# mokemokechicken/reversi-alpha-zero

Measured on NVIDIA H100. Metric: self_play_games_per_sec, higher is better.
Workload: dtype f16

## Files before the change

### reversi-alpha-zero_b200/csrc/rz_net_tc.cu

```cuda
#include <stdlib.h>
#include <type_traits>
#include "rz_bitboard.cuh"
#include "rz_net.cuh"
#include "rz_tc_common.cuh"

namespace rz {
namespace tc {

constexpr uint32_t kProducerRegs = 40, kMathRegs = 232;
constexpr int kMathThreads = 256;
constexpr uint32_t kActCg = 2896, kActSlot = 144;
constexpr uint32_t kActBytes = 32 * kActCg;
constexpr uint32_t kStageBytes = 32768, kStages = 3;
constexpr int kResAhead = 4;
constexpr uint32_t kA0Bytes = 8192, kW0Bytes = 16384;
constexpr uint32_t kOffAct = 0;
constexpr uint32_t kOffW = kOffAct + kActBytes;
constexpr uint32_t kOffA0 = kOffW + kStages * kStageBytes;
constexpr uint32_t kOffW0 = kOffA0 + kA0Bytes;
constexpr uint32_t kOffSS = kOffW0 + kW0Bytes;
constexpr uint32_t kOffHw = kOffSS + 2 * 2048;
constexpr uint32_t kOffBar = kOffHw + 768 * 4;
constexpr uint32_t kNumBars = 2 * kStages + 1;
constexpr uint32_t kSmemBytes = kOffBar + kNumBars * 8;
constexpr uint32_t kSmemAlloc = kSmemBytes + 128;
static_assert(kSmemAlloc <= 232448, "shared memory budget exceeded");
static_assert(kTowerResFloatsPerCta == (size_t)kMathThreads * 128, "residual scratch per CTA");

#ifdef RZ_TOWER_STAMPS
enum : int {
    kStTiles,
    kStTile,
    kStKLoop,
    kStFull,
    kStMma,
    kStEpiBar,
    kStEpi0,
    kStEpi1,
    kStEpi2,
    kStEpiLast,
    kStFeat,
    kStEmpty,
    kStCount
};
constexpr int kStMaxCtas = 1024;
__device__ unsigned long long g_tower_stamps[kStMaxCtas][kStCount];
__device__ __forceinline__ void stamp_add(int phase, uint32_t cycles) { atomicAdd(&g_tower_stamps[blockIdx.x][phase], (unsigned long long)cycles); }
#define RZ_STAMP(...) __VA_ARGS__
#else
#define RZ_STAMP(...)
#endif

template <int CL>
__global__ void __launch_bounds__(kThreads, 1) net_tower_kernel(const Params pp) {
    Params p = pp;
    if (p.n_dev) p.n = *p.n_dev;
    extern __shared__ uint8_t smem_raw[];
    const uint32_t base = (smem_u32(smem_raw) + 127u) & ~127u;
    uint8_t* sm = smem_raw + (base - smem_u32(smem_raw));
    const int warp = threadIdx.x >> 5, lane = threadIdx.x & 31;
    const uint32_t bar0 = base + kOffBar;
    auto bar_full = [&](uint32_t s) { return bar0 + s * 8; };
    auto bar_empty = [&](uint32_t s) { return bar0 + (kStages + s) * 8; };
    const uint32_t bar_w0 = bar0 + 2 * kStages * 8;
    const uint32_t ntiles = (p.n + 1) >> 1;
    const int L = p.n_layers;
    const uint32_t crank = CL > 1 ? cluster_ctarank() : 0u;
    const uint32_t cbase = blockIdx.x - crank;
    const uint32_t iters = cbase < ntiles ? (ntiles - cbase + gridDim.x - 1) / gridDim.x : 0u;

    for (uint32_t i = threadIdx.x * 16; i < kActBytes; i += kThreads * 16) *reinterpret_cast<uint4*>(sm + kOffAct + i) = make_uint4(0, 0, 0, 0);
    fence_proxy_async();
    for (uint32_t i = threadIdx.x; i < 768; i += kThreads)
        reinterpret_cast<float*>(sm + kOffHw)[i] = __ldg(i < 512 ? p.blob + p.off_policy_conv + i : p.blob + p.off_value_conv + (i - 512));
    if (threadIdx.x == 0) {
        for (uint32_t s = 0; s < kStages; ++s) { mbar_init(bar_full(s), 1); mbar_init(bar_empty(s), 8 * CL); }
        mbar_init(bar_w0, 1);
        asm volatile("fence.mbarrier_init.release.cluster;" ::: "memory");
    }
    __syncthreads();
    if (CL > 1) cluster_sync_all();

    if (warp >= 8) {
        asm volatile("setmaxnreg.dec.sync.aligned.u32 %0;" ::"n"(kProducerRegs));
        if (warp == 8 && lane == 0) {
            if (iters > 0) {
                mbar_expect_tx(bar_w0, kW0Bytes);
                bulk_g2s(base + kOffW0, p.w0, kW0Bytes, bar_w0);
            }
            uint32_t stage = 0, phase = 0;
            for (uint32_t it = 0; it < iters; ++it) {
                for (int l = 1; l < L; ++l) {
                    const uint8_t* src = reinterpret_cast<const uint8_t*>(p.w) + (size_t)(l - 1) * 36 * kStageBytes;
                    RZ_STAMP(uint32_t st_empty = 0;)
                    for (int s = 0; s < 36; ++s) {
                        RZ_STAMP(const uint32_t c0 = (uint32_t)clock();)
                        mbar_wait(bar_empty(stage), phase ^ 1);
                        RZ_STAMP(st_empty += (uint32_t)clock() - c0;)
                        mbar_expect_tx(bar_full(stage), kStageBytes);
                        if (CL == 1) {
                            bulk_g2s(base + kOffW + stage * kStageBytes, src + (size_t)s * kStageBytes, kStageBytes, bar_full(stage));
                        } else {
                            constexpr uint32_t kSlice = kStageBytes / CL;
                            bulk_g2s_mc(base + kOffW + stage * kStageBytes + crank * kSlice, src + (size_t)s * kStageBytes + crank * kSlice,
                                        kSlice, bar_full(stage), (uint16_t)((1u << CL) - 1u));
                        }
                        if (++stage == kStages) { stage = 0; phase ^= 1; }
                    }
                    RZ_STAMP(stamp_add(kStEmpty, st_empty);)
                }
            }
        }
    } else {
        asm volatile("setmaxnreg.inc.sync.aligned.u32 %0;" ::"n"(kMathRegs));
        const int et = threadIdx.x;
        const int wg = warp >> 2;
        const int r0 = wg * 64 + (warp & 3) * 16 + (lane >> 2);
        const int g0 = r0 >> 3, x = r0 & 7, y = g0 >> 1;
        const int cq = 2 * (lane & 3);
        const uint32_t act_row0 = base + kOffAct + (g0 + 2) * kActSlot + (x + 1) * 16 + cq * 2;
        const uint32_t act_row1 = act_row0 + kActSlot;
        const uint32_t a_wg = base + kOffAct + wg * 8 * kActSlot;
        float* ss_s = reinterpret_cast<float*>(sm + kOffSS);
        float4* res = reinterpret_cast<float4*>(p.res + (size_t)blockIdx.x * kTowerResFloatsPerCta) + et;
        const float* hw = reinterpret_cast<const float*>(sm + kOffHw);
        uint32_t stage = 0, phase = 0, ss_buf = 0;
        float d[128];
        ss_s[et] = __ldg(p.ss + et);
        ss_s[256 + et] = __ldg(p.ss + 256 + et);

        for (uint32_t it = 0; it < iters; ++it) {
            const uint32_t tile = blockIdx.x + it * gridDim.x;
            const uint32_t pos0 = tile * 2;
            RZ_STAMP(const uint32_t st_tile0 = (uint32_t)clock();)
            {
                const int m = et & 127, g = m >> 3, brd = g & 1;
                const bool valid = pos0 + brd < p.n;
                build_layer0_operand(sm + kOffA0, valid ? p.own[pos0 + brd] : 0, valid ? p.enemy[pos0 + brd] : 0, 2 * (et >> 7), g, m & 7,
                                     g >> 1);
                fence_proxy_async();
            }
            float hs[6];
            for (int l = 0; l < L; ++l) {
                const float* sc = ss_s + ss_buf * 512;
                const bool is_conv2 = l > 0 && (l & 1) == 0;
                float4 rb[kResAhead];
                RZ_STAMP(uint32_t st_c = (uint32_t)clock(), st_bar = 0, st_full = 0, st_mma = 0;)
                epi_bar();
                RZ_STAMP(st_bar += (uint32_t)clock() - st_c;)
                {
                    const size_t nl = l + 1 < L ? (size_t)l + 1 : 0;
                    const uint32_t dst = smem_u32(ss_s + (ss_buf ^ 1) * 512 + et);
                    cp_async_4(dst, p.ss + nl * 512 + et);
                    cp_async_4(dst + 1024, p.ss + nl * 512 + 256 + et);
                }
                RZ_STAMP(const uint32_t st_k0 = (uint32_t)clock();)
                acc_fence(d);
                if (l == 0) {
                    RZ_STAMP(st_c = (uint32_t)clock();)
                    mbar_wait(bar_w0, 0);
                    RZ_STAMP(st_full += (uint32_t)clock() - st_c;)
                    wgmma_fence();
#pragma unroll
                    for (uint32_t j = 0; j < 2; ++j)
                        wgmma_m64n256k16(d, smem_desc(base + kOffA0 + j * 2 * 2048 + wg * 1024, 2048, 128),
                                         smem_desc(base + kOffW0 + j * 2 * 4096, 4096, 128), j);
                    wgmma_commit();
                    RZ_STAMP(st_c = (uint32_t)clock();)
                    wgmma_wait<0>();
                    RZ_STAMP(st_mma += (uint32_t)clock() - st_c;)
                } else {
                    int prev = -1;
                    for (uint32_t tap = 0; tap < 9; ++tap) {
                        const uint32_t a_tap = a_wg + (2 * (tap / 3)) * kActSlot + (tap % 3) * 16;
                        for (uint32_t kb = 0; kb < 4; ++kb) {
                            RZ_STAMP(st_c = (uint32_t)clock();)
                            mbar_wait(bar_full(stage), phase);
                            RZ_STAMP(st_full += (uint32_t)clock() - st_c;)
                            const uint32_t b_st = base + kOffW + stage * kStageBytes;
                            wgmma_fence();
#pragma unroll
                            for (uint32_t j = 0; j < 4; ++j)
                                wgmma_m64n256k16(d, smem_desc(a_tap + (kb * 8 + 2 * j) * kActCg, kActCg, kActSlot),
                                                 smem_desc(b_st + 2 * j * 4096, 4096, 128), (tap | kb | j) != 0);
                            wgmma_commit();
                            RZ_STAMP(st_c = (uint32_t)clock();)
                            wgmma_wait<1>();
                            RZ_STAMP(st_mma += (uint32_t)clock() - st_c;)
                            if (prev >= 0 && lane == 0) {
                                mbar_arrive(bar_empty(prev));
                                if (CL > 1) mbar_arrive_cta(bar_empty(prev), crank ^ 1u);
                            }
                            prev = (int)stage;
                            if (++stage == kStages) { stage = 0; phase ^= 1; }
                        }
                    }
                    if (is_conv2) {
#pragma unroll
                        for (int i = 0; i < kResAhead; ++i) rb[i] = res[i * 256];
                    }
                    RZ_STAMP(st_c = (uint32_t)clock();)
                    wgmma_wait<0>();
                    RZ_STAMP(st_mma += (uint32_t)clock() - st_c;)
                    if (lane == 0) {
                        mbar_arrive(bar_empty(prev));
                        if (CL > 1) mbar_arrive_cta(bar_empty(prev), crank ^ 1u);
                    }
                }
                RZ_STAMP(const uint32_t st_k1 = (uint32_t)clock();)
                acc_fence(d);
                cp_async_wait_all();
                ss_buf ^= 1;
                const bool keep_res = l == 0 || is_conv2;
                const bool last = l == L - 1;
                RZ_STAMP(st_c = (uint32_t)clock();)
                if (!last) epi_bar();
                RZ_STAMP(const uint32_t st_e0 = (uint32_t)clock(); st_bar += st_e0 - st_c;)
                float* dbg0 = nullptr;
                float* dbg1 = nullptr;
                if (last && p.dbg_tower) {
                    if (pos0 < p.n) dbg0 = p.dbg_tower + ((size_t)pos0 * 64 + y * 8 + x) * 256;
                    if (pos0 + 1 < p.n) dbg1 = p.dbg_tower + ((size_t)(pos0 + 1) * 64 + y * 8 + x) * 256;
                }
                constexpr int kEpiRelu = 0, kEpiKeep = 1, kEpiLast = 2;
                auto epilogue = [&](auto conv2, auto kind) {
                    constexpr bool kConv2 = decltype(conv2)::value;
                    constexpr bool kKeep = decltype(kind)::value == kEpiKeep, kLast = decltype(kind)::value == kEpiLast;
                    if (kLast) {
#pragma unroll
                        for (int k = 0; k < 6; ++k) hs[k] = 0.f;
                    }
#pragma unroll
                for (int i = 0; i < 32; ++i) {
                    const int c = 8 * i + cq;
                    const float2 s = *reinterpret_cast<const float2*>(sc + c);
                    const float2 b = *reinterpret_cast<const float2*>(sc + 256 + c);
                    float v0 = fmaf(d[4 * i + 0], s.x, b.x), v1 = fmaf(d[4 * i + 1], s.y, b.y);
                    float v2 = fmaf(d[4 * i + 2], s.x, b.x), v3 = fmaf(d[4 * i + 3], s.y, b.y);
                    if (kConv2) {
                        const float4 r = rb[i % kResAhead];
                        if (i + kResAhead < 32) rb[i % kResAhead] = res[(i + kResAhead) * 256];
                        v0 += r.x; v1 += r.y; v2 += r.z; v3 += r.w;
                    }
                    if (kKeep || kLast) {
                        v0 = fmaxf(v0, 0.f); v1 = fmaxf(v1, 0.f); v2 = fmaxf(v2, 0.f); v3 = fmaxf(v3, 0.f);
                    }
                    if (!kLast) {
                        if (kKeep) res[i * 256] = make_float4(v0, v1, v2, v3);
                        const uint32_t h0 = pack_h2<!kKeep>(v0, v1);
                        const uint32_t h1 = pack_h2<!kKeep>(v2, v3);
                        const uint32_t off = (c >> 3) * kActCg;
                        asm volatile("st.shared.b32 [%0], %1;" ::"r"(act_row0 + off), "r"(h0) : "memory");
                        asm volatile("st.shared.b32 [%0], %1;" ::"r"(act_row1 + off), "r"(h1) : "memory");
                    } else {
                        const float4 w = *reinterpret_cast<const float4*>(hw + 2 * c);
                        const float2 wv = *reinterpret_cast<const float2*>(hw + 512 + c);
                        hs[0] = fmaf(v1, w.z, fmaf(v0, w.x, hs[0]));
                        hs[1] = fmaf(v1, w.w, fmaf(v0, w.y, hs[1]));
                        hs[2] = fmaf(v1, wv.y, fmaf(v0, wv.x, hs[2]));
                        hs[3] = fmaf(v3, w.z, fmaf(v2, w.x, hs[3]));
                        hs[4] = fmaf(v3, w.w, fmaf(v2, w.y, hs[4]));
                        hs[5] = fmaf(v3, wv.y, fmaf(v2, wv.x, hs[5]));
                        if (dbg0) *reinterpret_cast<float2*>(dbg0 + c) = make_float2(v0, v1);
                        if (dbg1) *reinterpret_cast<float2*>(dbg1 + c) = make_float2(v2, v3);
                    }
                }
                };
                using Conv2 = std::true_type;
                using NoConv2 = std::false_type;
                if (last) {
                    if (is_conv2) epilogue(Conv2(), std::integral_constant<int, kEpiLast>());
                    else epilogue(NoConv2(), std::integral_constant<int, kEpiLast>());
                } else if (is_conv2) {
                    epilogue(Conv2(), std::integral_constant<int, kEpiKeep>());
                } else if (keep_res) {
                    epilogue(NoConv2(), std::integral_constant<int, kEpiKeep>());
                } else {
                    epilogue(NoConv2(), std::integral_constant<int, kEpiRelu>());
                }
                if (!last) fence_proxy_async();
                RZ_STAMP(if (et == 0) {
                    stamp_add(kStKLoop, st_k1 - st_k0); stamp_add(kStFull, st_full); stamp_add(kStMma, st_mma); stamp_add(kStEpiBar, st_bar);
                    stamp_add(l == 0 ? kStEpi0 : last ? kStEpiLast : is_conv2 ? kStEpi2 : kStEpi1, (uint32_t)clock() - st_e0);
                })
            }
            RZ_STAMP(const uint32_t st_h0 = (uint32_t)clock();)
#pragma unroll
            for (int k = 0; k < 6; ++k) {
                hs[k] += __shfl_xor_sync(0xffffffffu, hs[k], 1);
                hs[k] += __shfl_xor_sync(0xffffffffu, hs[k], 2);
            }
            {
                const int q = lane & 3;
                if (q < 2 && pos0 + q < p.n) {
                    const float h0 = q ? hs[3] : hs[0], h1 = q ? hs[4] : hs[1], h2 = q ? hs[5] : hs[2];
                    store_head_features(p.feat + (size_t)(pos0 + q) * kHeadFeatures, p.ss + (size_t)L * 512, y * 8 + x, h0 + 0.f,
                                        h1 + 0.f, h2 + 0.f);
                }
            }
            RZ_STAMP(if (et == 0) {
                const uint32_t st_h1 = (uint32_t)clock();
                stamp_add(kStFeat, st_h1 - st_h0); stamp_add(kStTile, st_h1 - st_tile0); stamp_add(kStTiles, 1);
            })
        }
    }

    __syncthreads();
    if (CL > 1) cluster_sync_all();
}

int launch_tower(const Params& p, cudaStream_t stream) {
    return launch_tower_pairs<net_tower_kernel<1>, net_tower_kernel<2>, kSmemAlloc, 2>(p, stream);
}

}

static int g_cluster = 0;

int set_tower_cluster(int cluster) {
    RZ_REQUIRE(cluster == 1 || cluster == 2, "rz_net_set_tower_cluster: cluster must be 1 or 2");
    g_cluster = cluster;
    return RZ_OK;
}

int tower_cluster() {
    if (g_cluster == 0) {
        const char* cs = getenv("RZ_TOWER_CLUSTER");
        g_cluster = (cs && atoi(cs) == 1) ? 1 : 2;
    }
    return g_cluster;
}

}

#ifdef RZ_TOWER_STAMPS
extern "C" int rz_tower_stamps(unsigned long long* out, int n_ctas, int reset) {
    using namespace rz::tc;
    if (n_ctas < 0 || n_ctas > kStMaxCtas) return (int)cudaErrorInvalidValue;
    const size_t bytes = (size_t)n_ctas * kStCount * sizeof(unsigned long long);
    cudaError_t e = cudaDeviceSynchronize();
    if (e == cudaSuccess && out) e = cudaMemcpyFromSymbol(out, g_tower_stamps, bytes);
    if (e == cudaSuccess && reset) {
        void* dev = nullptr;
        e = cudaGetSymbolAddress(&dev, g_tower_stamps);
        if (e == cudaSuccess) e = cudaMemset(dev, 0, sizeof(g_tower_stamps));
        if (e == cudaSuccess) e = cudaDeviceSynchronize();
    }
    return (int)e;
}
extern "C" int rz_tower_stamp_count() { return rz::tc::kStCount; }
#endif
```

### reversi-alpha-zero_b200/csrc/rz_tc_common.cuh

```cuda
#pragma once
#include <cuda_fp16.h>
#include "rz_bitboard.cuh"
#include "rz_net.cuh"

namespace rz {
namespace tc {

__device__ __forceinline__ uint32_t smem_u32(const void* p) { return (uint32_t)__cvta_generic_to_shared(p); }

__device__ __forceinline__ void mbar_init(uint32_t bar, uint32_t count) {
    asm volatile("mbarrier.init.shared::cta.b64 [%0], %1;" ::"r"(bar), "r"(count) : "memory");
}
__device__ __forceinline__ void mbar_expect_tx(uint32_t bar, uint32_t bytes) {
    asm volatile("mbarrier.arrive.expect_tx.shared::cta.b64 _, [%0], %1;" ::"r"(bar), "r"(bytes) : "memory");
}
__device__ __forceinline__ void mbar_arrive(uint32_t bar) {
    asm volatile("mbarrier.arrive.shared::cta.b64 _, [%0];" ::"r"(bar) : "memory");
}
__device__ __forceinline__ void mbar_arrive_cta(uint32_t bar, uint32_t rank) {
    uint32_t remote;
    asm volatile("mapa.shared::cluster.u32 %0, %1, %2;" : "=r"(remote) : "r"(bar), "r"(rank));
    asm volatile("mbarrier.arrive.shared::cluster.b64 _, [%0];" ::"r"(remote) : "memory");
}
__device__ __forceinline__ void mbar_wait(uint32_t bar, uint32_t parity) {
    uint32_t ok = 0;
    long long t0 = 0;
    for (uint32_t spin = 0; !ok; ++spin) {
        asm volatile(
            "{\n\t.reg .pred p;\n\t"
            "mbarrier.try_wait.parity.shared::cta.b64 p, [%1], %2;\n\t"
            "selp.u32 %0, 1, 0, p;\n\t}"
            : "=r"(ok)
            : "r"(bar), "r"(parity)
            : "memory");
        if (!ok && (spin & 1023) == 1023) {
            const long long now = clock64();
            if (t0 == 0) t0 = now;
            else if (now - t0 > 8000000000LL) __trap();
        }
    }
}
__device__ __forceinline__ void bulk_g2s(uint32_t dst, const void* src, uint32_t bytes, uint32_t bar) {
    asm volatile("cp.async.bulk.shared::cluster.global.mbarrier::complete_tx::bytes [%0], [%1], %2, [%3];" ::"r"(dst), "l"(src),
                 "r"(bytes), "r"(bar)
                 : "memory");
}
__device__ __forceinline__ void bulk_g2s_mc(uint32_t dst, const void* src, uint32_t bytes, uint32_t bar, uint16_t mask) {
    asm volatile(
        "cp.async.bulk.shared::cluster.global.mbarrier::complete_tx::bytes.multicast::cluster [%0], [%1], %2, [%3], %4;" ::"r"(dst),
        "l"(src), "r"(bytes), "r"(bar), "h"(mask)
        : "memory");
}
__device__ __forceinline__ void cluster_sync_all() {
    asm volatile("barrier.cluster.arrive.release.aligned;\n\tbarrier.cluster.wait.acquire.aligned;" ::: "memory");
}
__device__ __forceinline__ uint32_t cluster_ctarank() {
    uint32_t r;
    asm volatile("mov.u32 %0, %%cluster_ctarank;" : "=r"(r));
    return r;
}
__device__ __forceinline__ void cp_async_4(uint32_t dst, const void* src) {
    asm volatile("cp.async.ca.shared.global [%0], [%1], 4;" ::"r"(dst), "l"(src) : "memory");
}
__device__ __forceinline__ void cp_async_wait_all() { asm volatile("cp.async.wait_all;" ::: "memory"); }
__device__ __forceinline__ void fence_proxy_async() { asm volatile("fence.proxy.async.shared::cta;" ::: "memory"); }
__device__ __forceinline__ void epi_bar() { asm volatile("bar.sync 1, 256;" ::: "memory"); }

__device__ __forceinline__ uint64_t smem_desc(uint32_t addr, uint32_t lbo, uint32_t sbo) {
    return (uint64_t)((addr >> 4) & 0x3FFF) | ((uint64_t)((lbo >> 4) & 0x3FFF) << 16) | ((uint64_t)((sbo >> 4) & 0x3FFF) << 32);
}
__device__ __forceinline__ void wgmma_fence() { asm volatile("wgmma.fence.sync.aligned;" ::: "memory"); }
__device__ __forceinline__ void wgmma_commit() { asm volatile("wgmma.commit_group.sync.aligned;" ::: "memory"); }
template <int N>
__device__ __forceinline__ void wgmma_wait() { asm volatile("wgmma.wait_group.sync.aligned %0;" ::"n"(N) : "memory"); }
__device__ __forceinline__ void acc_fence(float (&d)[128]) {
#pragma unroll
    for (int i = 0; i < 128; ++i) asm volatile("" : "+f"(d[i])::"memory");
}

#define RZ_D4(i) "+f"(d[i]), "+f"(d[i + 1]), "+f"(d[i + 2]), "+f"(d[i + 3])
#define RZ_D16(i) RZ_D4(i), RZ_D4(i + 4), RZ_D4(i + 8), RZ_D4(i + 12)
__device__ __forceinline__ void wgmma_m64n256k16(float (&d)[128], uint64_t adesc, uint64_t bdesc, uint32_t accumulate) {
    asm volatile(
        "{\n\t.reg .pred p;\n\t"
        "setp.ne.b32 p, %130, 0;\n\t"
        "wgmma.mma_async.sync.aligned.m64n256k16.f32.f16.f16 {"
        "%0, %1, %2, %3, %4, %5, %6, %7, %8, %9, %10, %11, %12, %13, %14, %15, "
        "%16, %17, %18, %19, %20, %21, %22, %23, %24, %25, %26, %27, %28, %29, %30, %31, "
        "%32, %33, %34, %35, %36, %37, %38, %39, %40, %41, %42, %43, %44, %45, %46, %47, "
        "%48, %49, %50, %51, %52, %53, %54, %55, %56, %57, %58, %59, %60, %61, %62, %63, "
        "%64, %65, %66, %67, %68, %69, %70, %71, %72, %73, %74, %75, %76, %77, %78, %79, "
        "%80, %81, %82, %83, %84, %85, %86, %87, %88, %89, %90, %91, %92, %93, %94, %95, "
        "%96, %97, %98, %99, %100, %101, %102, %103, %104, %105, %106, %107, %108, %109, %110, %111, "
        "%112, %113, %114, %115, %116, %117, %118, %119, %120, %121, %122, %123, %124, %125, %126, %127"
        "}, %128, %129, p, 1, 1, 0, 0;\n\t}"
        : RZ_D16(0), RZ_D16(16), RZ_D16(32), RZ_D16(48), RZ_D16(64), RZ_D16(80), RZ_D16(96), RZ_D16(112)
        : "l"(adesc), "l"(bdesc), "r"(accumulate)
        : "memory");
}
template <int O>
__device__ __forceinline__ void wgmma_m64n128k16(float (&d)[128], uint64_t adesc, uint64_t bdesc, uint32_t accumulate) {
    asm volatile(
        "{\n\t.reg .pred p;\n\t"
        "setp.ne.b32 p, %66, 0;\n\t"
        "wgmma.mma_async.sync.aligned.m64n128k16.f32.f16.f16 {"
        "%0, %1, %2, %3, %4, %5, %6, %7, %8, %9, %10, %11, %12, %13, %14, %15, "
        "%16, %17, %18, %19, %20, %21, %22, %23, %24, %25, %26, %27, %28, %29, %30, %31, "
        "%32, %33, %34, %35, %36, %37, %38, %39, %40, %41, %42, %43, %44, %45, %46, %47, "
        "%48, %49, %50, %51, %52, %53, %54, %55, %56, %57, %58, %59, %60, %61, %62, %63"
        "}, %64, %65, p, 1, 1, 0, 0;\n\t}"
        : RZ_D16(O), RZ_D16(O + 16), RZ_D16(O + 32), RZ_D16(O + 48)
        : "l"(adesc), "l"(bdesc), "r"(accumulate)
        : "memory");
}
template <int O>
__device__ __forceinline__ void wgmma_m64n64k16(float (&d)[128], uint64_t adesc, uint64_t bdesc, uint32_t accumulate) {
    asm volatile(
        "{\n\t.reg .pred p;\n\t"
        "setp.ne.b32 p, %34, 0;\n\t"
        "wgmma.mma_async.sync.aligned.m64n64k16.f32.f16.f16 {"
        "%0, %1, %2, %3, %4, %5, %6, %7, %8, %9, %10, %11, %12, %13, %14, %15, "
        "%16, %17, %18, %19, %20, %21, %22, %23, %24, %25, %26, %27, %28, %29, %30, %31"
        "}, %32, %33, p, 1, 1, 0, 0;\n\t}"
        : RZ_D16(O), RZ_D16(O + 16)
        : "l"(adesc), "l"(bdesc), "r"(accumulate)
        : "memory");
}
#undef RZ_D16
#undef RZ_D4

template <bool RELU>
__device__ __forceinline__ uint32_t pack_h2(float a, float b) {
    uint32_t d;
    if (RELU) asm("cvt.rn.relu.satfinite.f16x2.f32 %0, %1, %2;" : "=r"(d) : "f"(b), "f"(a));
    else      asm("cvt.rn.satfinite.f16x2.f32 %0, %1, %2;" : "=r"(d) : "f"(b), "f"(a));
    return d;
}

struct Params {
    const __half* w0;
    const __half* w;
    const float* ss;
    const float* blob;
    size_t off_policy_conv, off_policy_fc_k, off_policy_fc_b, off_value_conv, off_value_fc1_k, off_value_fc1_b, off_value_fc2_k,
        off_value_fc2_b;
    const u64* own;
    const u64* enemy;
    float* policy;
    float* value;
    float* res;
    float* feat;
    float* dbg_tower;
    float* dbg_logits;
    float* dbg_vlogit;
    uint32_t n;
    const uint32_t* n_dev;
    int n_layers;
    int V;
};

constexpr uint32_t kTcMaxV = 512;

constexpr int kThreads = 384;

template <void (*K1)(Params), void (*K2)(Params), uint32_t kSmem, uint32_t kBoards>
int launch_tower_pairs(const Params& p, cudaStream_t stream) {
    static int max_pairs = -1;
    if (max_pairs < 0) {
        RZ_CUDA_TRY(cudaFuncSetAttribute(K1, cudaFuncAttributeMaxDynamicSharedMemorySize, (int)kSmem));
        RZ_CUDA_TRY(cudaFuncSetAttribute(K2, cudaFuncAttributeMaxDynamicSharedMemorySize, (int)kSmem));
        cudaLaunchConfig_t cfg = {};
        cfg.gridDim = dim3((unsigned)num_sms() & ~1u); cfg.blockDim = dim3(kThreads); cfg.dynamicSmemBytes = kSmem;
        cudaLaunchAttribute attr[1];
        attr[0].id = cudaLaunchAttributeClusterDimension;
        attr[0].val.clusterDim.x = 2; attr[0].val.clusterDim.y = 1; attr[0].val.clusterDim.z = 1;
        cfg.attrs = attr; cfg.numAttrs = 1;
        RZ_CUDA_TRY(cudaOccupancyMaxActiveClusters(&max_pairs, K2, &cfg));
    }
    const int cluster = tower_cluster() == 2 && max_pairs >= 1 ? 2 : 1;
    const uint32_t ntiles = (p.n + kBoards - 1) / kBoards;
    uint32_t grid = ntiles < (uint32_t)num_sms() ? ntiles : (uint32_t)num_sms();
    if (cluster == 1) {
        K1<<<grid, kThreads, kSmem, stream>>>(p);
    } else {
        grid = (grid + 1) & ~1u;
        if (grid > 2u * (uint32_t)max_pairs) grid = 2u * (uint32_t)max_pairs;
        cudaLaunchConfig_t cfg = {};
        cfg.gridDim = dim3(grid); cfg.blockDim = dim3(kThreads); cfg.dynamicSmemBytes = kSmem; cfg.stream = stream;
        cudaLaunchAttribute attr[1];
        attr[0].id = cudaLaunchAttributeClusterDimension;
        attr[0].val.clusterDim.x = 2; attr[0].val.clusterDim.y = 1; attr[0].val.clusterDim.z = 1;
        cfg.attrs = attr; cfg.numAttrs = 1;
        RZ_CUDA_TRY(cudaLaunchKernelEx(&cfg, K2, p));
    }
    RZ_LAUNCH_CHECK();
    return RZ_OK;
}

int launch_tower(const Params& p, cudaStream_t stream);
int launch_tower_narrow(const Params& p, int filters, cudaStream_t stream);
int launch_tower_split(const Params& p, cudaStream_t stream);

__device__ __forceinline__ void build_layer0_operand(uint8_t* a0, u64 o, u64 e, int kc0, int g, int x, int y) {
#pragma unroll
    for (int kk = 0; kk < 2; ++kk) {
        const int kc = kc0 + kk;
        uint32_t w[4];
#pragma unroll
        for (int jp = 0; jp < 4; ++jp) {
            uint32_t packed = 0;
#pragma unroll
            for (int half = 0; half < 2; ++half) {
                const int k = kc * 8 + jp * 2 + half;
                uint32_t bit = 0;
                if (k < 18) {
                    const int tap = k >> 1, yy = y + tap / 3 - 1, xx = x + tap % 3 - 1;
                    if (yy >= 0 && yy < 8 && xx >= 0 && xx < 8) bit = (uint32_t)((((k & 1) ? e : o) >> (yy * 8 + xx)) & 1ULL);
                }
                packed |= (bit ? 0x3C00u : 0u) << (16 * half);
            }
            w[jp] = packed;
        }
        *reinterpret_cast<uint4*>(a0 + kc * 2048 + g * 128 + x * 16) = make_uint4(w[0], w[1], w[2], w[3]);
    }
}

__device__ __forceinline__ void store_head_features(float* f, const float* ssh, int pix, float a0, float a1, float av) {
    f[pix] = fmaxf(fmaf(a0, ssh[0], ssh[2]), 0.f);
    f[64 + pix] = fmaxf(fmaf(a1, ssh[1], ssh[3]), 0.f);
    f[128 + pix] = fmaxf(fmaf(av, ssh[4], ssh[5]), 0.f);
}

}

int net_heads(const tc::Params& p, cudaStream_t stream);

}
```

Measured before the change: 24.91.

## Transpose conv tower GEMM so weights are A and activations are B

```diff
diff --git a/reversi-alpha-zero_b200/csrc/rz_net_tc.cu b/reversi-alpha-zero_b200/csrc/rz_net_tc.cu
--- a/reversi-alpha-zero_b200/csrc/rz_net_tc.cu
+++ b/reversi-alpha-zero_b200/csrc/rz_net_tc.cu
@@ -13,6 +13,11 @@
 constexpr uint32_t kActBytes = 32 * kActCg;
 constexpr uint32_t kStageBytes = 32768, kStages = 3;
 constexpr int kResAhead = 4;
+constexpr uint32_t kStgRow = 260, kStgBytes = 64 * kStgRow * 4;
+constexpr uint32_t kStgCgs = (kStgBytes + kActCg - 1) / kActCg;
+constexpr uint32_t kBorderChunks = 18 + 17;
+static_assert(kStgBytes <= kActBytes, "staging exceeds the operand buffer");
+__device__ constexpr int last_order(int j) { return (j & 8) * 2 + (j >> 4) * 8 + (j & 7); }
 constexpr uint32_t kA0Bytes = 8192, kW0Bytes = 16384;
 constexpr uint32_t kOffAct = 0;
 constexpr uint32_t kOffW = kOffAct + kActBytes;
@@ -115,12 +120,11 @@
         asm volatile("setmaxnreg.inc.sync.aligned.u32 %0;" ::"n"(kMathRegs));
         const int et = threadIdx.x;
         const int wg = warp >> 2;
-        const int r0 = wg * 64 + (warp & 3) * 16 + (lane >> 2);
-        const int g0 = r0 >> 3, x = r0 & 7, y = g0 >> 1;
+        const int c0 = wg * 128 + (warp & 3) * 16 + (lane >> 2);
         const int cq = 2 * (lane & 3);
-        const uint32_t act_row0 = base + kOffAct + (g0 + 2) * kActSlot + (x + 1) * 16 + cq * 2;
-        const uint32_t act_row1 = act_row0 + kActSlot;
-        const uint32_t a_wg = base + kOffAct + wg * 8 * kActSlot;
+        const uint32_t st_row = base + kOffAct + (wg * 16 + (warp & 3) * 2 + ((lane >> 3) & 1)) * kActCg + ((lane >> 4) + 2) * kActSlot +
+                                ((lane & 7) + 1) * 16;
+        float* stg = reinterpret_cast<float*>(sm + kOffAct);
         float* ss_s = reinterpret_cast<float*>(sm + kOffSS);
         float4* res = reinterpret_cast<float4*>(p.res + (size_t)blockIdx.x * kTowerResFloatsPerCta) + et;
         const float* hw = reinterpret_cast<const float*>(sm + kOffHw);
@@ -162,37 +166,52 @@
                     RZ_STAMP(st_full += (uint32_t)clock() - st_c;)
                     wgmma_fence();
 #pragma unroll
-                    for (uint32_t j = 0; j < 2; ++j)
-                        wgmma_m64n256k16(d, smem_desc(base + kOffA0 + j * 2 * 2048 + wg * 1024, 2048, 128),
-                                         smem_desc(base + kOffW0 + j * 2 * 4096, 4096, 128), j);
+                    for (uint32_t j = 0; j < 2; ++j) {
+                        const uint32_t a = base + kOffW0 + j * 2 * 4096 + wg * 2048;
+                        const uint64_t b = smem_desc(base + kOffA0 + j * 2 * 2048, 2048, 128);
+                        wgmma_m64n128k16<0>(d, smem_desc(a, 4096, 128), b, j);
+                        wgmma_m64n128k16<64>(d, smem_desc(a + 1024, 4096, 128), b, j);
+                    }
                     wgmma_commit();
                     RZ_STAMP(st_c = (uint32_t)clock();)
                     wgmma_wait<0>();
                     RZ_STAMP(st_mma += (uint32_t)clock() - st_c;)
                 } else {
                     int prev = -1;
-                    for (uint32_t tap = 0; tap < 9; ++tap) {
-                        const uint32_t a_tap = a_wg + (2 * (tap / 3)) * kActSlot + (tap % 3) * 16;
-                        for (uint32_t kb = 0; kb < 4; ++kb) {
-                            RZ_STAMP(st_c = (uint32_t)clock();)
-                            mbar_wait(bar_full(stage), phase);
-                            RZ_STAMP(st_full += (uint32_t)clock() - st_c;)
-                            const uint32_t b_st = base + kOffW + stage * kStageBytes;
-                            wgmma_fence();
-#pragma unroll
-                            for (uint32_t j = 0; j < 4; ++j)
-                                wgmma_m64n256k16(d, smem_desc(a_tap + (kb * 8 + 2 * j) * kActCg, kActCg, kActSlot),
-                                                 smem_desc(b_st + 2 * j * 4096, 4096, 128), (tap | kb | j) != 0);
-                            wgmma_commit();
-                            RZ_STAMP(st_c = (uint32_t)clock();)
-                            wgmma_wait<1>();
-                            RZ_STAMP(st_mma += (uint32_t)clock() - st_c;)
-                            if (prev >= 0 && lane == 0) {
-                                mbar_arrive(bar_empty(prev));
-                                if (CL > 1) mbar_arrive_cta(bar_empty(prev), crank ^ 1u);
+#pragma unroll
+                    for (uint32_t kh = 0; kh < 3; ++kh) {
+                        for (uint32_t kw = 0; kw < 3; ++kw) {
+                            const uint64_t b_tap = smem_desc(base + kOffAct + 2 * kh * kActSlot + kw * 16, kActCg, kActSlot);
+                            for (uint32_t kb = 0; kb < 4; ++kb) {
+                                RZ_STAMP(st_c = (uint32_t)clock();)
+                                mbar_wait(bar_full(stage), phase);
+                                RZ_STAMP(st_full += (uint32_t)clock() - st_c;)
+                                const uint64_t a_st = smem_desc(base + kOffW + stage * kStageBytes + wg * 2048, 4096, 128);
+                                const uint64_t b_kb = b_tap + kb * 8 * (kActCg >> 4);
+                                wgmma_fence();
+#pragma unroll
+                                for (uint32_t j = 0; j < 4; ++j) {
+                                    const uint64_t a0 = a_st + j * (2 * 4096 >> 4), a1 = a0 + (1024 >> 4), b = b_kb + j * (2 * kActCg >> 4);
+                                    const uint32_t acc = (kh | kw | kb | j) != 0;
+                                    if (kh == 2) {
+                                        wgmma_m64n112k16<0>(d, a0, b, acc);
+                                        wgmma_m64n112k16<64>(d, a1, b, acc);
+                                    } else {
+                                        wgmma_m64n128k16<0>(d, a0, b, acc);
+                                        wgmma_m64n128k16<64>(d, a1, b, acc);
+                                    }
+                                }
+                                wgmma_commit();
+                                RZ_STAMP(st_c = (uint32_t)clock();)
+                                wgmma_wait<1>();
+                                RZ_STAMP(st_mma += (uint32_t)clock() - st_c;)
+                                if (prev >= 0 && lane == 0) {
+                                    mbar_arrive(bar_empty(prev));
+                                    if (CL > 1) mbar_arrive_cta(bar_empty(prev), crank ^ 1u);
+                                }
+                                prev = (int)stage;
+                                if (++stage == kStages) { stage = 0; phase ^= 1; }
                             }
-                            prev = (int)stage;
-                            if (++stage == kStages) { stage = 0; phase ^= 1; }
                         }
                     }
                     if (is_conv2) {
@@ -214,32 +233,55 @@
                 const bool keep_res = l == 0 || is_conv2;
                 const bool last = l == L - 1;
                 RZ_STAMP(st_c = (uint32_t)clock();)
-                if (!last) epi_bar();
+                epi_bar();
                 RZ_STAMP(const uint32_t st_e0 = (uint32_t)clock(); st_bar += st_e0 - st_c;)
-                float* dbg0 = nullptr;
-                float* dbg1 = nullptr;
-                if (last && p.dbg_tower) {
-                    if (pos0 < p.n) dbg0 = p.dbg_tower + ((size_t)pos0 * 64 + y * 8 + x) * 256;
-                    if (pos0 + 1 < p.n) dbg1 = p.dbg_tower + ((size_t)(pos0 + 1) * 64 + y * 8 + x) * 256;
-                }
+                if (l == 0 && !last) {
+                    for (uint32_t k = et; k < kStgCgs * kBorderChunks; k += kMathThreads) {
+                        const uint32_t r = k % kBorderChunks;
+                        *reinterpret_cast<uint4*>(sm + kOffAct + (k / kBorderChunks) * kActCg + (r < 18 ? r * 16 : (r - 16) * kActSlot)) =
+                            make_uint4(0, 0, 0, 0);
+                    }
+                }
+                auto head_half = [&](int h) {
+                    const int m = et >> 2, n = 64 * h + m, brd = (m >> 3) & 1;
+                    const float* row = stg + m * kStgRow + cq;
+                    float* dbg = p.dbg_tower && pos0 + brd < p.n
+                                     ? p.dbg_tower + ((size_t)(pos0 + brd) * 64 + (n >> 4) * 8 + (n & 7)) * 256 + cq
+                                     : nullptr;
+                    float a0 = 0.f, a1 = 0.f, av = 0.f;
+#pragma unroll
+                    for (int i = 0; i < 32; ++i) {
+                        const int c = 8 * i + cq;
+                        const float2 v = *reinterpret_cast<const float2*>(row + 8 * i);
+                        const float4 w = *reinterpret_cast<const float4*>(hw + 2 * c);
+                        const float2 wv = *reinterpret_cast<const float2*>(hw + 512 + c);
+                        a0 = fmaf(v.y, w.z, fmaf(v.x, w.x, a0));
+                        a1 = fmaf(v.y, w.w, fmaf(v.x, w.y, a1));
+                        av = fmaf(v.y, wv.y, fmaf(v.x, wv.x, av));
+                        if (dbg) *reinterpret_cast<float2*>(dbg + 8 * i) = v;
+                    }
+                    hs[3 * h] = a0; hs[3 * h + 1] = a1; hs[3 * h + 2] = av;
+                };
                 constexpr int kEpiRelu = 0, kEpiKeep = 1, kEpiLast = 2;
                 auto epilogue = [&](auto conv2, auto kind) {
                     constexpr bool kConv2 = decltype(conv2)::value;
                     constexpr bool kKeep = decltype(kind)::value == kEpiKeep, kLast = decltype(kind)::value == kEpiLast;
-                    if (kLast) {
-#pragma unroll
-                        for (int k = 0; k < 6; ++k) hs[k] = 0.f;
-                    }
-#pragma unroll
-                for (int i = 0; i < 32; ++i) {
-                    const int c = 8 * i + cq;
-                    const float2 s = *reinterpret_cast<const float2*>(sc + c);
-                    const float2 b = *reinterpret_cast<const float2*>(sc + 256 + c);
-                    float v0 = fmaf(d[4 * i + 0], s.x, b.x), v1 = fmaf(d[4 * i + 1], s.y, b.y);
-                    float v2 = fmaf(d[4 * i + 2], s.x, b.x), v3 = fmaf(d[4 * i + 3], s.y, b.y);
+                    float s[4], t[4];
+#pragma unroll
+                    for (int k = 0; k < 4; ++k) {
+                        s[k] = sc[c0 + 64 * (k >> 1) + 8 * (k & 1)];
+                        t[k] = sc[256 + c0 + 64 * (k >> 1) + 8 * (k & 1)];
+                    }
+                    uint32_t hp0 = 0, hp1 = 0;
+#pragma unroll
+                for (int j = 0; j < 32; ++j) {
+                    const int i = kLast ? last_order(j) : j;
+                    const int b = i >> 4, ii = i & 15;
+                    float v0 = fmaf(d[4 * i + 0], s[2 * b], t[2 * b]), v1 = fmaf(d[4 * i + 1], s[2 * b], t[2 * b]);
+                    float v2 = fmaf(d[4 * i + 2], s[2 * b + 1], t[2 * b + 1]), v3 = fmaf(d[4 * i + 3], s[2 * b + 1], t[2 * b + 1]);
                     if (kConv2) {
-                        const float4 r = rb[i % kResAhead];
-                        if (i + kResAhead < 32) rb[i % kResAhead] = res[(i + kResAhead) * 256];
+                        const float4 r = rb[j % kResAhead];
+                        if (j + kResAhead < 32) rb[j % kResAhead] = res[(kLast ? last_order(j + kResAhead) : j + kResAhead) * 256];
                         v0 += r.x; v1 += r.y; v2 += r.z; v3 += r.w;
                     }
                     if (kKeep || kLast) {
@@ -249,20 +291,16 @@
                         if (kKeep) res[i * 256] = make_float4(v0, v1, v2, v3);
                         const uint32_t h0 = pack_h2<!kKeep>(v0, v1);
                         const uint32_t h1 = pack_h2<!kKeep>(v2, v3);
-                        const uint32_t off = (c >> 3) * kActCg;
-                        asm volatile("st.shared.b32 [%0], %1;" ::"r"(act_row0 + off), "r"(h0) : "memory");
-                        asm volatile("st.shared.b32 [%0], %1;" ::"r"(act_row1 + off), "r"(h1) : "memory");
+                        if (ii & 1) stmatrix_x4_trans(st_row + 8 * b * kActCg + (ii - 1) * kActSlot, hp0, hp1, h0, h1);
+                        else { hp0 = h0; hp1 = h1; }
                     } else {
-                        const float4 w = *reinterpret_cast<const float4*>(hw + 2 * c);
-                        const float2 wv = *reinterpret_cast<const float2*>(hw + 512 + c);
-                        hs[0] = fmaf(v1, w.z, fmaf(v0, w.x, hs[0]));
-                        hs[1] = fmaf(v1, w.w, fmaf(v0, w.y, hs[1]));
-                        hs[2] = fmaf(v1, wv.y, fmaf(v0, wv.x, hs[2]));
-                        hs[3] = fmaf(v3, w.z, fmaf(v2, w.x, hs[3]));
-                        hs[4] = fmaf(v3, w.w, fmaf(v2, w.y, hs[4]));
-                        hs[5] = fmaf(v3, wv.y, fmaf(v2, wv.x, hs[5]));
-                        if (dbg0) *reinterpret_cast<float2*>(dbg0 + c) = make_float2(v0, v1);
-                        if (dbg1) *reinterpret_cast<float2*>(dbg1 + c) = make_float2(v2, v3);
+                        float* o = stg + (8 * (ii & 7) + cq) * kStgRow + c0 + 64 * b;
+                        o[0] = v0; o[kStgRow] = v1; o[8] = v2; o[kStgRow + 8] = v3;
+                        if ((j & 15) == 15) {
+                            epi_bar();
+                            head_half(j >> 4);
+                            if (j == 15) epi_bar();
+                        }
                     }
                 }
                 };
@@ -290,12 +328,13 @@
                 hs[k] += __shfl_xor_sync(0xffffffffu, hs[k], 1);
                 hs[k] += __shfl_xor_sync(0xffffffffu, hs[k], 2);
             }
-            {
-                const int q = lane & 3;
-                if (q < 2 && pos0 + q < p.n) {
-                    const float h0 = q ? hs[3] : hs[0], h1 = q ? hs[4] : hs[1], h2 = q ? hs[5] : hs[2];
-                    store_head_features(p.feat + (size_t)(pos0 + q) * kHeadFeatures, p.ss + (size_t)L * 512, y * 8 + x, h0 + 0.f,
-                                        h1 + 0.f, h2 + 0.f);
+            if ((lane & 3) == 0) {
+#pragma unroll
+                for (int h = 0; h < 2; ++h) {
+                    const int m = et >> 2, n = 64 * h + m, brd = (m >> 3) & 1;
+                    if (pos0 + brd < p.n)
+                        store_head_features(p.feat + (size_t)(pos0 + brd) * kHeadFeatures, p.ss + (size_t)L * 512, (n >> 4) * 8 + (n & 7),
+                                            hs[3 * h] + 0.f, hs[3 * h + 1] + 0.f, hs[3 * h + 2] + 0.f);
                 }
             }
             RZ_STAMP(if (et == 0) {
diff --git a/reversi-alpha-zero_b200/csrc/rz_tc_common.cuh b/reversi-alpha-zero_b200/csrc/rz_tc_common.cuh
--- a/reversi-alpha-zero_b200/csrc/rz_tc_common.cuh
+++ b/reversi-alpha-zero_b200/csrc/rz_tc_common.cuh
@@ -114,6 +114,21 @@
         : "memory");
 }
 template <int O>
+__device__ __forceinline__ void wgmma_m64n112k16(float (&d)[128], uint64_t adesc, uint64_t bdesc, uint32_t accumulate) {
+    asm volatile(
+        "{\n\t.reg .pred p;\n\t"
+        "setp.ne.b32 p, %58, 0;\n\t"
+        "wgmma.mma_async.sync.aligned.m64n112k16.f32.f16.f16 {"
+        "%0, %1, %2, %3, %4, %5, %6, %7, %8, %9, %10, %11, %12, %13, %14, %15, "
+        "%16, %17, %18, %19, %20, %21, %22, %23, %24, %25, %26, %27, %28, %29, %30, %31, "
+        "%32, %33, %34, %35, %36, %37, %38, %39, %40, %41, %42, %43, %44, %45, %46, %47, "
+        "%48, %49, %50, %51, %52, %53, %54, %55"
+        "}, %56, %57, p, 1, 1, 0, 0;\n\t}"
+        : RZ_D16(O), RZ_D16(O + 16), RZ_D16(O + 32), RZ_D4(O + 48), RZ_D4(O + 52)
+        : "l"(adesc), "l"(bdesc), "r"(accumulate)
+        : "memory");
+}
+template <int O>
 __device__ __forceinline__ void wgmma_m64n64k16(float (&d)[128], uint64_t adesc, uint64_t bdesc, uint32_t accumulate) {
     asm volatile(
         "{\n\t.reg .pred p;\n\t"
@@ -128,6 +143,12 @@
 }
 #undef RZ_D16
 #undef RZ_D4
+
+__device__ __forceinline__ void stmatrix_x4_trans(uint32_t addr, uint32_t r0, uint32_t r1, uint32_t r2, uint32_t r3) {
+    asm volatile("stmatrix.sync.aligned.m8n8.x4.trans.shared.b16 [%0], {%1, %2, %3, %4};" ::"r"(addr), "r"(r0), "r"(r1), "r"(r2),
+                 "r"(r3)
+                 : "memory");
+}
 
 template <bool RELU>
 __device__ __forceinline__ uint32_t pack_h2(float a, float b) {
```

Measured after the change: 25.53, median of 6. 1.02x the previous value.
